# bababyVN/medical-image-segmentation-and-classification

Hardware: NVIDIA B200
Metric: AttU_Net 256x256 train images/sec (higher is better)
Workload: dtype bf16

## Files before the change

### include/b200seg.h

```cpp
#ifndef B200SEG_H_
#define B200SEG_H_

#include <stdint.h>

#ifdef __cplusplus
extern "C" {
#endif

#define B2_ABI_VERSION 1

enum {
  B2_OK = 0,
  B2_ERR_SHAPE = -1,
  B2_ERR_ALIGN = -2,
  B2_ERR_ARCH = -3,
  B2_ERR_CUDA = -4,
  B2_ERR_NCCL = -5,
  B2_ERR_WORKSPACE = -6
};

typedef void* b2_stream_t;

const char* b2_last_error(void);
int b2_abi_version(void);
int b2_arch_check(void);
int b2_num_sms(void);

int b2_set_deterministic(void* workspace, int64_t bytes);
int b2_get_deterministic(void);

int b2_reload_env(void);

typedef struct b2_conv_args {
  int32_t n, h, w;
  int32_t ksize;
  const void* x0;
  int32_t c0, ldx0;
  const void* x1;
  int32_t c1, ldx1;
  const void* wpk;
  int32_t ktot;
  int64_t w_tap_stride;
  int32_t cout;
  void* y;
  int32_t ldy;
  const float* bias;
  const void* addend;
  int32_t ldadd;
  double* stats;
  int32_t relu;
  int32_t stride;
  int32_t out_mul, out_off_h, out_off_w;
  int32_t in_mul, in_off_h, in_off_w;
  int32_t custom_pad, pad_h, pad_w;
  int32_t add_after_act;
  int32_t fold_mode;
} b2_conv_args;

int b2_conv_fprop(const b2_conv_args* a, b2_stream_t stream);
int b2_conv_dgrad(const b2_conv_args* a, b2_stream_t stream);

typedef struct b2_wgrad_args {
  int32_t n, h, w;
  int32_t ksize;
  const void* dy;
  int32_t cout, lddy;
  const void* x0;
  int32_t c0, ldx0;
  const void* x1;
  int32_t c1, ldx1;
  float* dw;
  int32_t accumulate;
  void* workspace;
  int64_t workspace_bytes;
  int32_t x_stride;
  int32_t dy_mul, dy_off_h, dy_off_w;
  int32_t custom_pad, pad_h, pad_w;
  int32_t fold;
} b2_wgrad_args;

int64_t b2_conv_wgrad_workspace(const b2_wgrad_args* a);
int b2_conv_wgrad(const b2_wgrad_args* a, b2_stream_t stream);
// ... 206 lines not shown
```

### medical-image-segmentation-and-classification_b200/b200seg/_lib.py

```python
from __future__ import annotations

import ctypes as C
import os
from pathlib import Path

_PKG_DIR = Path(__file__).resolve().parent
LIB_PATH = Path(os.environ.get("B200SEG_LIB", _PKG_DIR.parent / "lib" / "libb200seg.so"))

B2_OK = 0
ERR_NAMES = {-1: "B2_ERR_SHAPE", -2: "B2_ERR_ALIGN", -3: "B2_ERR_ARCH", -4: "B2_ERR_CUDA", -5: "B2_ERR_NCCL",
             -6: "B2_ERR_WORKSPACE"}

_vp, _i32, _i64, _f32 = C.c_void_p, C.c_int32, C.c_int64, C.c_float


class ConvArgs(C.Structure):
    _fields_ = [("n", _i32), ("h", _i32), ("w", _i32), ("ksize", _i32),
                ("x0", _vp), ("c0", _i32), ("ldx0", _i32),
                ("x1", _vp), ("c1", _i32), ("ldx1", _i32),
                ("wpk", _vp), ("ktot", _i32), ("w_tap_stride", _i64),
                ("cout", _i32), ("y", _vp), ("ldy", _i32),
                ("bias", _vp), ("addend", _vp), ("ldadd", _i32),
                ("stats", _vp), ("relu", _i32),
                ("stride", _i32), ("out_mul", _i32), ("out_off_h", _i32), ("out_off_w", _i32),
                ("in_mul", _i32), ("in_off_h", _i32), ("in_off_w", _i32),
                ("custom_pad", _i32), ("pad_h", _i32), ("pad_w", _i32), ("add_after_act", _i32),
                ("fold_mode", _i32)]


class WgradArgs(C.Structure):
    _fields_ = [("n", _i32), ("h", _i32), ("w", _i32), ("ksize", _i32),
                ("dy", _vp), ("cout", _i32), ("lddy", _i32),
                ("x0", _vp), ("c0", _i32), ("ldx0", _i32),
                ("x1", _vp), ("c1", _i32), ("ldx1", _i32),
                ("dw", _vp), ("accumulate", _i32),
                ("workspace", _vp), ("workspace_bytes", _i64), ("x_stride", _i32),
                ("dy_mul", _i32), ("dy_off_h", _i32), ("dy_off_w", _i32),
                ("custom_pad", _i32), ("pad_h", _i32), ("pad_w", _i32), ("fold", _i32)]


class BnRunRef(C.Structure):
    _fields_ = [("stats", _vp), ("running_mean", _vp), ("running_var", _vp), ("num_batches_tracked", _vp),
                ("count", _i64), ("c", _i32), ("momentum", C.c_float)]


class F32ConvArgs(C.Structure):
    _fields_ = [("x0", _vp), ("x1", _vp), ("c0", _i32), ("c1", _i32), ("ldx0", _i32), ("ldx1", _i32),
                ("n", _i32), ("hi", _i32), ("wi", _i32), ("ho", _i32), ("wo", _i32),
                ("ksize", _i32), ("stride", _i32), ("pad_h", _i32), ("pad_w", _i32),
                ("w", _vp), ("bias", _vp), ("addend", _vp),
                ("ldadd", _i32), ("add_after_act", _i32), ("relu", _i32), ("cout", _i32),
                ("y", _vp), ("ldy", _i32), ("out_mul", _i32), ("out_off_h", _i32), ("out_off_w", _i32)]


class GateArgs(C.Structure):
    _fields_ = [("n", _i32), ("h", _i32), ("w", _i32), ("c", _i32), ("fint", _i32),
                ("g", _vp), ("ldg", _i32), ("x", _vp), ("ldx", _i32),
                ("wpk", _vp), ("bias", _vp), ("wpsi", _vp), ("bpsi", _vp), ("scale1", _vp), ("shift1", _vp),
                ("out", _vp), ("ldo", _i32)]


class GateCoef(C.Structure):
    _fields_ = [(k, _vp) for k in (
        "scale_g", "shift_g", "mean_g", "invstd_g", "gamma_g",
        "scale_x", "shift_x", "mean_x", "invstd_x", "gamma_x",
        "gamma1", "mean1", "invstd1", "wpsi")]


SIGNATURES = {
    "b2_last_error": (C.c_char_p, []),
    "b2_abi_version": (C.c_int, []),
    "b2_arch_check": (C.c_int, []),
    "b2_num_sms": (C.c_int, []),
    "b2_set_deterministic": (C.c_int, [_vp, _i64]),
    "b2_get_deterministic": (C.c_int, []),
    "b2_reload_env": (C.c_int, []),
    "b2_conv_fprop": (C.c_int, [C.POINTER(ConvArgs), _vp]),
    "b2_conv_dgrad": (C.c_int, [C.POINTER(ConvArgs), _vp]),
    "b2_conv_wgrad_workspace": (_i64, [C.POINTER(WgradArgs)]),
    "b2_conv_wgrad": (C.c_int, [C.POINTER(WgradArgs), _vp]),
    "b2_pack_weights": (C.c_int, [_vp, _i32, _i32, _i32, _i64, _i64, _i64, _i64, _vp, _vp, _vp]),
    "b2_pack_weights_folded": (C.c_int, [_vp, _i32, _i32, _i32, _i64, _i64, _i64, _i64, _vp, _vp, _vp, _i32, _vp, _vp,
                                         _vp]),
    "b2_pack_weights_upfold": (C.c_int, [_vp, _i32, _i32, _i64, _i64, _i64, _i64, _vp, _vp, _vp]),
    "b2_fold_upconv_wgrad": (C.c_int, [_vp, _i32, _i32, _vp, _vp]),
    "b2_conv_smallc_fprop": (C.c_int, [_vp, _i32, _i32, _i32, _i32, _vp, _vp, _i32, _vp, _i32, _i32, _vp]),
    "b2_conv_smallc_wgrad": (C.c_int, [_vp, _i32, _vp, _i32, _i32, _i32, _i32, _i32, _vp, _vp]),
    "b2_head_fwd": (C.c_int, [_vp, _i32, _i64, _i32, _i32, _vp, _vp, _i32, _vp, _vp]),
    "b2_head_bwd": (C.c_int, [_vp, _vp, _i32, _i64, _i32, _i32, _vp, _i32, _vp, _i32, _vp, _vp, _vp]),
    "b2_channel_stats": (C.c_int, [_vp, _i32, _i64, _i32, _vp, _vp]),
    "b2_bn_finalize": (C.c_int, [_vp, _i32, _i64, _vp, _vp, _f32, _f32, _vp, _vp, _vp, _vp, _vp, _vp, _vp, _vp]),
    "b2_bn_update_running_multi": (C.c_int, [_vp, _i32, _i32, _vp]),
    "b2_bn_eval_coeffs": (C.c_int, [_vp, _vp, _vp, _vp, _f32, _i32, _vp, _vp, _vp, _vp, _vp]),
    "b2_bn_apply": (C.c_int, [_vp, _i32, _i64, _i32, _vp, _vp, _i32, _vp, _i32, _vp, _i32, _vp, _i32, _vp]),
    "b2_bn_bwd_reduce": (C.c_int, [_vp, _i32, _vp, _i32, _i64, _i32, _vp, _vp, _vp, _vp, _i32, _vp, _vp]),
    "b2_bn_bwd_apply": (C.c_int, [_vp, _i32, _vp, _i32, _i64, _i32, _vp, _vp, _vp, _vp, _vp, _i32, _i32, _vp,
                                  _vp, _i32, _vp, _vp, _vp, _vp]),
    "b2_channel_sum": (C.c_int, [_vp, _i32, _i64, _i32, _vp, _vp]),
    "b2_maxpool2x2_fwd": (C.c_int, [_vp, _i32, _i32, _i32, _i32, _i32, _vp, _i32, _vp]),
    "b2_maxpool2x2_bwd": (C.c_int, [_vp, _i32, _vp, _i32, _i32, _i32, _i32, _i32, _vp, _i32, _vp]),
    "b2_maxpool2x2_bwd_add": (C.c_int, [_vp, _i32, _vp, _i32, _i32, _i32, _i32, _i32, _vp, _i32, _vp, _i32, _vp]),
    "b2_upsample2x_fwd": (C.c_int, [_vp, _i32, _i32, _i32, _i32, _i32, _vp, _i32, _vp]),
    "b2_upsample2x_bwd": (C.c_int, [_vp, _i32, _i32, _i32, _i32, _i32, _vp, _i32, _vp]),
    "b2_add": (C.c_int, [_vp, _i32, _vp, _i32, _i64, _i32, _vp, _i32, _vp]),
    "b2_nchw_f32_to_nhwc_bf16": (C.c_int, [_vp, _i32, _i32, _i32, _i32, _vp, _i32, _vp]),
    "b2_stem_im2col3x3": (C.c_int, [_vp, _i32, _i32, _i32, _i32, _vp, _vp]),
    "b2_layout_nchw_to_nhwc": (C.c_int, [_vp, _i32, _i32, _i32, _i32, _vp, _i32, _vp]),
    "b2_layout_nhwc_to_nchw": (C.c_int, [_vp, _i32, _i32, _i32, _i32, _i32, _vp, _vp]),
    "b2_stem7x7_fprop": (C.c_int, [_vp, _i32, _i32, _i32, _vp, _i32, _vp, _i32, _vp]),
    "b2_maxpool3x3s2_fwd": (C.c_int, [_vp, _i32, _i32, _i32, _i32, _i32, _vp, _i32, _vp]),
    "b2_gate_psi_fwd": (C.c_int, [_vp, _vp, _i32, _i64, _i32, _vp, _vp, _vp, _vp, _vp, _vp, _vp, _vp, _vp]),
    "b2_gate_apply_fwd": (C.c_int, [_vp, _i32, _vp, _i64, _i32, _vp, _vp, _vp, _vp, _i32, _vp]),
    "b2_gate_apply_bwd": (C.c_int, [_vp, _i32, _vp, _i32, _vp, _vp, _i64, _i32, _vp, _vp, _vp, _i32, _vp, _vp,
                                    _vp]),
    "b2_gate_psi_bwd_reduce": (C.c_int, [_vp, _vp, _vp, _vp, _i32, _i64, _i32, C.POINTER(GateCoef), _vp, _i32,
                                         _vp, _vp, _vp, _vp]),
    "b2_gate_psi_bwd_apply": (C.c_int, [_vp, _vp, _vp, _vp, _i32, _i64, _i32, C.POINTER(GateCoef), _vp, _i32,
                                        _vp, _vp, _vp, _vp, _vp, _vp, _vp]),
    "b2_grad_sqnorm_multi": (C.c_int, [_vp, _vp, _vp, _i32, _i32, _vp, _vp, _vp]),
    "b2_adamw_multi": (C.c_int, [_vp, _vp, _vp, _i32, _i32, _vp, _f32, _vp, _f32, _f32, _f32, _f32, _vp, _vp, _vp]),
    "b2_pack_weights_multi": (C.c_int, [_vp, _i32, _i32, _vp]),
    "b2_seg_augment": (C.c_int, [_vp, _vp, _i32, _i32, _i32, _i32, _vp, C.POINTER(_f32), C.POINTER(_f32), _i32, _vp, _vp,
                                 _vp]),
    "b2_gate_fused": (C.c_int, [C.POINTER(GateArgs), _vp]),
    "b2_stem_im2col": (C.c_int, [_vp, _i32, _i32, _i32, _i32, _i32, _i32, _i32, _i32, _vp, _vp]),
    "b2_maxpool3x3s2_bwd": (C.c_int, [_vp, _i32, _vp, _i32, _i32, _i32, _i32, _i32, _vp, _i32, _vp]),
    "b2_zero_insert2x": (C.c_int, [_vp, _i32, _i32, _i32, _i32, _i32, _vp, _i32, _vp]),
# ... 66 lines not shown
```

### medical-image-segmentation-and-classification_b200/csrc/common.cuh

```cuda
#pragma once
#include <cuda.h>
#include <cuda_runtime.h>
#include <cuda_bf16.h>
#include <stdint.h>
#include <stdio.h>
#include <string.h>

#include "../../include/b200seg.h"

namespace b2 {

void set_error(const char* fmt, ...);
int  cuda_fail(cudaError_t e, const char* what);

#define B2_CHECK_CUDA(expr)                                            \
  do {                                                                 \
    cudaError_t _e = (expr);                                           \
    if (_e != cudaSuccess) return ::b2::cuda_fail(_e, #expr);          \
  } while (0)

#define B2_REQUIRE(cond, code, ...)                                    \
  do {                                                                 \
    if (!(cond)) { ::b2::set_error(__VA_ARGS__); return (code); }      \
  } while (0)
// ... 4 lines not shown

int env_switch(const char* name, int dflt);

__device__ __forceinline__ void pdl_wait() { asm volatile("griddepcontrol.wait;" ::: "memory"); }
__device__ __forceinline__ void pdl_trigger() { asm volatile("griddepcontrol.launch_dependents;" ::: "memory"); }
__device__ __forceinline__ void pdl_enter() {
  pdl_wait();
  pdl_trigger();
}

inline bool pdl_allowed(long long work_bytes) {
  const int mode = env_switch("B200SEG_PDL", 2);
  if (mode == 0) return false;
  if (mode == 1) return true;
  return work_bytes <= (long long)env_switch("B200SEG_PDL_MB", 16) * (1ll << 20);
}

template <typename... KArgs, typename... Args>
inline cudaError_t launch_chain(void (*kernel)(KArgs...), dim3 grid, dim3 block, size_t smem, cudaStream_t stream,
                                int cluster, long long work_bytes, Args&&... args) {
  cudaLaunchConfig_t cfg = {};
  cfg.gridDim = grid;
  cfg.blockDim = block;
  cfg.dynamicSmemBytes = smem;
  cfg.stream = stream;
  cudaLaunchAttribute at[2];
  unsigned n = 0;
  if (cluster > 1) {
    at[n].id = cudaLaunchAttributeClusterDimension;
    at[n].val.clusterDim.x = (unsigned)cluster;
    at[n].val.clusterDim.y = 1;
    at[n].val.clusterDim.z = 1;
    ++n;
  }
  if (pdl_allowed(work_bytes)) {
    at[n].id = cudaLaunchAttributeProgrammaticStreamSerialization;
    at[n].val.programmaticStreamSerializationAllowed = 1;
    ++n;
  }
  cfg.attrs = at;
  cfg.numAttrs = n;
  return cudaLaunchKernelEx(&cfg, kernel, static_cast<KArgs>(args)...);
}

int encode_tmap_bf16(CUtensorMap* out, const void* base, int rank, const uint64_t* dims,
                     const uint64_t* strides_bytes, const uint32_t* box, CUtensorMapSwizzle swz,
                     const uint32_t* elem_strides = nullptr);

struct DetBuf {
  double* partial;
  int n;
};
int det_begin(DetBuf* out, long long rows, int n, cudaStream_t stream, long long keep = 0);
int det_finish(const double* partial, long long rows, int row_stride, int count, double* dst, cudaStream_t stream);
int det_finish(const double* partial, long long rows, int row_stride, int count, float* dst, cudaStream_t stream);
bool det_enabled();

#ifdef __CUDACC__
template <typename T>
__device__ __forceinline__ void red_out(T* dst, const DetBuf& d, int idx, T v) {
  if (d.partial != nullptr) d.partial[(size_t)blockIdx.x * d.n + idx] = (double)v;
  else atomicAdd(dst + idx, v);
}
__device__ __forceinline__ uint32_t smem_u32(const void* p) {
  return (uint32_t)__cvta_generic_to_shared(p);
}

__device__ __forceinline__ void mbar_init(uint64_t* bar, uint32_t count) {
  asm volatile("mbarrier.init.shared::cta.b64 [%0], %1;" ::"r"(smem_u32(bar)), "r"(count) : "memory");
}
__device__ __forceinline__ void fence_barrier_init() {
  asm volatile("fence.mbarrier_init.release.cluster;" ::: "memory");
}
__device__ __forceinline__ void fence_proxy_async() {
  asm volatile("fence.proxy.async.shared::cta;" ::: "memory");
}
__device__ __forceinline__ void mbar_arrive_expect_tx(uint64_t* bar, uint32_t bytes) {
  asm volatile("mbarrier.arrive.expect_tx.shared::cta.b64 _, [%0], %1;" ::"r"(smem_u32(bar)), "r"(bytes)
               : "memory");
}
__device__ __forceinline__ void mbar_arrive(uint64_t* bar) {
  asm volatile("mbarrier.arrive.shared::cta.b64 _, [%0];" ::"r"(smem_u32(bar)) : "memory");
}
__device__ __forceinline__ bool mbar_try_wait(uint64_t* bar, uint32_t parity) {
  uint32_t ok;
  asm volatile(
      "{\n\t.reg .pred p;\n\t"
      "mbarrier.try_wait.parity.shared::cta.b64 p, [%1], %2;\n\t"
      "selp.u32 %0, 1, 0, p;\n\t}"
      : "=r"(ok)
      : "r"(smem_u32(bar)), "r"(parity)
      : "memory");
  return ok != 0;
}
__device__ __forceinline__ void mbar_wait(uint64_t* bar, uint32_t parity) {
  uint32_t spins = 0;
  while (!mbar_try_wait(bar, parity)) {
    if (++spins > (1u << 26)) { __trap(); }
  }
}

__device__ __forceinline__ void tma_load_2d(void* smem, const CUtensorMap* tm, uint64_t* bar, int c0, int c1) {
  asm volatile(
      "cp.async.bulk.tensor.2d.shared::cluster.global.mbarrier::complete_tx::bytes [%0], [%1, {%3, %4}], [%2];"
      ::"r"(smem_u32(smem)), "l"(reinterpret_cast<uint64_t>(tm)), "r"(smem_u32(bar)), "r"(c0), "r"(c1)
      : "memory");
// ... 227 lines not shown
```

### medical-image-segmentation-and-classification_b200/csrc/conv_igemm.cu

```cuda
#include <stdlib.h>
#include <mutex>

#include "common.cuh"
#include "igemm_util.cuh"

namespace b2 {

static constexpr int kMaxEpiGroups = 2;
static constexpr int kThreads = 64 + 128 * kMaxEpiGroups;
static constexpr int kMaxStages = 12;

struct IgemmParams {
  int H, W, N;
  int Wb, Hb, Nb;
  int tw, th;
  int taps;
  int cb0, cb1;
  int block_n, stages, num_k_iters;
  int cout, n_tiles, m_tiles, m_stride;
  int halo, base_off_mode;
  int dm;
  int rp;
  int stride, ksize, pad_h, pad_w;
  long long y_sn, y_sh, y_sw;
// ... 290 lines not shown
#pragma unroll
                  for (int k = 0; k < kKBlock / 16; ++k)
                    umma_bf16(d_tmem, desc_hi | (uint64_t)(a_lo + 2 * k), desc_hi | (uint64_t)(b_lo + 2 * k), idesc,
                              (it | s | k) != 0 ? 1u : 0u);
                }
                a_lo += 8;
                b_lo += b_tap_step;
              }
            }
          } else {
          const uint32_t d_tmem = tmem_base + (uint32_t)((ti & 1) * p.block_n);
          for (int s = 0; s < ((p.debug_skip & 2) ? 0 : sub); ++s) {
            const uint32_t a_s = a_addr + s * 128;
            const uint32_t b_s = b_addr + s * p.block_n * 128;
            const uint32_t bo = p.base_off_mode ? ((a_s >> 7) & 7u) : 0u;
#pragma unroll
            for (int k = 0; k < kKBlock / 16; ++k) {
              const uint64_t da = umma_desc_sw128_bo(a_s + k * 32, 16, 1024, bo);
              const uint64_t db = umma_desc_sw128(b_s + k * 32, 16, 1024);
              umma_bf16(d_tmem, da, db, idesc, (it | s | k) != 0 ? 1u : 0u);
            }
          }
          }
          if constexpr (kPair) {
            umma_commit_pair(&empty_bar[stage], 3);
          } else {
            if (C == 1) umma_commit(&empty_bar[stage]);
            else umma_commit_mc(&empty_bar[stage], cmask);
          }
        }
        __syncwarp();
        if (++stage == p.stages) {
          stage = 0;
          phase ^= 1;
        }
      }
      if (elect_one()) {
        for (int q = 0; q < a_slots; ++q) {
          uint64_t* fb = &tmem_full_bar[(uint32_t)(a_slots * ti + q) & (uint32_t)(nbuf - 1)];
          if constexpr (kPair) umma_commit_pair(fb, 3);
          else umma_commit(fb);
        }
      }
      __syncwarp();
    }
  } else if (warp >= 2 && ((warp - 2) >> 2) < p.epi_groups) {
    const int g = (warp - 2) >> 2;
    const int G = p.epi_groups;
    const int et = (threadIdx.x - 64) & 127;
    uint8_t* ctile = ctile0 + g * ctile_bytes;
    float* s_bias = s_bias0 + g * 256;
    float* s_psi = s_psi0 + g * 256;
    const int bar_id = 1 + g;
    const int quad = warp & 3;
    const int row = quad * 32 + lane;
    const int wl = row % p.Wb;
    const int hl = (row / p.Wb) % p.Hb;
    const int nl = row / (p.Wb * p.Hb);
    const bool relu = p.relu != 0;
    const int nchunks = p.block_n >> 3;
    const int schunk = lane % nchunks;
    const int sgrp = et / nchunks;
    double acc[16];
#pragma unroll
    for (int i = 0; i < 16; ++i) acc[i] = 0.0;
    const int fold_tiles = 32 / nchunks;
    float fs[8], fq[8];
#pragma unroll
    for (int j = 0; j < 8; ++j) fs[j] = fq[j] = 0.f;
    int fpending = 0;
    auto fold_stats = [&]() {
#pragma unroll
      for (int j = 0; j < 8; ++j) {
        acc[j] += (double)fs[j];
        acc[8 + j] += (double)fq[j];
        fs[j] = fq[j] = 0.f;
      }
      fpending = 0;
    };

    auto flush_stats = [&](int n_tile_) {
      fold_stats();
      for (int off = nchunks; off < 32; off <<= 1) {
#pragma unroll
        for (int i = 0; i < 16; ++i) acc[i] += __shfl_xor_sync(0xffffffffu, acc[i], off);
      }
      if (p.tma_store && et == 0) tma_store_wait_read();
      asm volatile("bar.sync %0, 128;" ::"r"(bar_id) : "memory");
      double* red = reinterpret_cast<double*>(ctile);
      if (lane < nchunks) {
        double* r0 = red + ((warp - 2) & 3) * 2 * p.block_n + schunk * 8;
#pragma unroll
        for (int j = 0; j < 8; ++j) {
          r0[j] = acc[j];
          r0[p.block_n + j] = acc[8 + j];
        }
      }
      asm volatile("bar.sync %0, 128;" ::"r"(bar_id) : "memory");
      for (int i = et; i < 2 * p.block_n; i += 128) {
        const int which = i / p.block_n, c = i % p.block_n;
        double v = 0.0;
#pragma unroll
        for (int w = 0; w < 4; ++w) v += red[(w * 2 + which) * p.block_n + c];
        const int sidx = which * p.cout + n_tile_ * p.block_n + (p.rp ? (c & 63) : c);
        if (p.stats_partial != nullptr)
          p.stats_partial[(size_t)(blockIdx.x * p.epi_groups + g) * (2 * p.cout) + sidx] += v;
// ... 740 lines not shown
```

### medical-image-segmentation-and-classification_b200/csrc/conv_small.cu

```cuda
#include "common.cuh"

namespace b2 {

template <int KS>
__global__ void __launch_bounds__(128) smallc_fprop_kernel(const uint2* __restrict__ x4, int n, int h, int w,
                                                           const float* __restrict__ wk,
                                                           const float* __restrict__ bias, int cout,
                                                           __nv_bfloat16* __restrict__ y, int ldy, int relu) {
  constexpr int TAPS = KS * KS;
  extern __shared__ float sm[];
  float* sw = sm;
  float* sb = sm + cout * TAPS * 4;
  for (int i = threadIdx.x; i < cout * TAPS * 4; i += blockDim.x) sw[i] = bf16_round(wk[i]);
  for (int i = threadIdx.x; i < cout; i += blockDim.x) sb[i] = bias ? bias[i] : 0.f;
  __syncthreads();
  const long long total = (long long)n * h * w;
  for (long long p = (long long)blockIdx.x * blockDim.x + threadIdx.x; p < total;
       p += (long long)gridDim.x * blockDim.x) {
    const int xx = (int)(p % w);
    const int yy = (int)((p / w) % h);
    float in[TAPS][4];
#pragma unroll
    for (int t = 0; t < TAPS; ++t) {
      const int dy = (KS == 3) ? t / 3 - 1 : 0, dx = (KS == 3) ? t % 3 - 1 : 0;
// ... 287 lines not shown
    smallc_wgrad_kernel<3><<<(unsigned)grid, 256, 0, (cudaStream_t)stream>>>((const __nv_bfloat16*)dy, lddy,
                                                                             (const uint2*)x4, n, h, w, dw, det);
  else
    smallc_wgrad_kernel<1><<<(unsigned)grid, 256, 0, (cudaStream_t)stream>>>((const __nv_bfloat16*)dy, lddy,
                                                                             (const uint2*)x4, n, h, w, dw, det);
  B2_LAUNCH_CHECK();
  if (det.partial) return det_finish(det.partial, grid, det.n, ncol, dw, (cudaStream_t)stream);
  return B2_OK;
}

extern "C" int b2_head_fwd(const void* x, int32_t ldx, int64_t npix, int32_t hw, int32_t cin, const float* w,
                           const float* bias, int32_t cout, float* y, b2_stream_t stream) {
  B2_REQUIRE(cin % 8 == 0 && cin <= 256, B2_ERR_SHAPE, "head cin=%d must be a multiple of 8, <= 256", cin);
  B2_REQUIRE(cout >= 1 && cout <= 8, B2_ERR_SHAPE, "head cout=%d must be in 1..8", cout);
  B2_REQUIRE(npix > 0 && npix < (1ll << 31) && hw > 0, B2_ERR_SHAPE, "head: pixel count out of range");
  B2_REQUIRE(ldx % 8 == 0 && (reinterpret_cast<uintptr_t>(x) & 15) == 0, B2_ERR_ALIGN, "x misaligned");
  const int L = pow2ceil(cin / 8);
  const int gpb = 256 / L;
  long long grid = (npix + gpb - 1) / gpb;
  const long long cap = (long long)num_sms() * 8;
  if (grid > cap) grid = cap;
#define B2_HEAD_FWD(CO) head_fwd_kernel<CO><<<(unsigned)grid, 256, 0, (cudaStream_t)stream>>>( \
      (const __nv_bfloat16*)x, ldx, npix, hw, cin, w, bias, cout, L, y)
  if (cout == 1) B2_HEAD_FWD(1); else if (cout == 2) B2_HEAD_FWD(2); else if (cout <= 4) B2_HEAD_FWD(4); else B2_HEAD_FWD(8);
#undef B2_HEAD_FWD
  B2_LAUNCH_CHECK();
  return B2_OK;
}

extern "C" int b2_head_bwd(const float* dy, const void* x, int32_t ldx, int64_t npix, int32_t hw, int32_t cin,
                           const float* w, int32_t cout, void* dx, int32_t lddx, float* dw, float* db,
                           b2_stream_t stream) {
  B2_REQUIRE(cin % 8 == 0 && cin <= 256, B2_ERR_SHAPE, "head cin=%d must be a multiple of 8, <= 256", cin);
  B2_REQUIRE(cout >= 1 && cout <= 8, B2_ERR_SHAPE, "head cout=%d must be in 1..8", cout);
  B2_REQUIRE(npix > 0 && npix < (1ll << 31) && hw > 0, B2_ERR_SHAPE, "head: pixel count out of range");
  B2_REQUIRE(ldx % 8 == 0 && (reinterpret_cast<uintptr_t>(x) & 15) == 0, B2_ERR_ALIGN, "x misaligned");
  B2_REQUIRE(dx == nullptr || (lddx % 8 == 0 && (reinterpret_cast<uintptr_t>(dx) & 15) == 0), B2_ERR_ALIGN,
             "dx misaligned");
  const int L = pow2ceil(cin / 8);
  const int gpb = 256 / L;
  long long grid = (npix + gpb - 1) / gpb;
  const long long cap = (long long)num_sms() * 6;
  if (grid > cap) grid = cap;
  const size_t smem = (size_t)(cout * cin + cout) * sizeof(float);
  DetBuf det;
  int rc = det_begin(&det, grid, cout * cin + cout, (cudaStream_t)stream);
  if (rc) return rc;
#define B2_HEAD_BWD(CO) head_bwd_kernel<CO><<<(unsigned)grid, 256, smem, (cudaStream_t)stream>>>( \
      dy, (const __nv_bfloat16*)x, ldx, npix, hw, cin, w, cout, L, (__nv_bfloat16*)dx, lddx, dw, db, det)
  if (cout == 1) B2_HEAD_BWD(1); else if (cout == 2) B2_HEAD_BWD(2); else if (cout <= 4) B2_HEAD_BWD(4); else B2_HEAD_BWD(8);
#undef B2_HEAD_BWD
  B2_LAUNCH_CHECK();
  if (det.partial) {
    rc = det_finish(det.partial, grid, det.n, cout * cin, dw, (cudaStream_t)stream);
    if (rc) return rc;
    return det_finish(det.partial + cout * cin, grid, det.n, cout, db, (cudaStream_t)stream);
  }
  return B2_OK;
}
```

### medical-image-segmentation-and-classification_b200/csrc/gate.cu

```cuda
#include <stdlib.h>

#include "common.cuh"

namespace b2 {

__device__ __forceinline__ void g_unpack8(const uint4& u, float* f) {
  f[0] = bf16lo(u.x); f[1] = bf16hi(u.x); f[2] = bf16lo(u.y); f[3] = bf16hi(u.y);
  f[4] = bf16lo(u.z); f[5] = bf16hi(u.z); f[6] = bf16lo(u.w); f[7] = bf16hi(u.w);
}
__device__ __forceinline__ uint4 g_pack8(const float* f) {
  return make_uint4(pack_bf16x2(f[0], f[1]), pack_bf16x2(f[2], f[3]), pack_bf16x2(f[4], f[5]),
                    pack_bf16x2(f[6], f[7]));
}
__device__ __forceinline__ void g_load8(const float* p, bool has, float* f) {
#pragma unroll
  for (int j = 0; j < 8; ++j) f[j] = has ? __ldg(p + j) : 0.f;
}
__device__ __forceinline__ float sigmoidf_(float x) { return 1.f / (1.f + expf(-x)); }

__device__ __forceinline__ void block_sum2_out(float a, float b, double* dst, const DetBuf& det) {
  __shared__ float sh[2][8];
  a = warp_sum(a);
  b = warp_sum(b);
  const int warp = threadIdx.x >> 5, lane = threadIdx.x & 31;
// ... 501 lines not shown
  B2_CHECK_CUDA(launch_chain(gate_apply_bwd_kernel, dim3(grid), dim3(256), (size_t)(0), (cudaStream_t)stream, 1,
      (long long)npix * c * 2, (const __nv_bfloat16*)dout, lddout, (const __nv_bfloat16*)x, ldx,
      (const __nv_bfloat16*)psi, (const __nv_bfloat16*)q, npix, c / 8, L, mean1, invstd1, (__nv_bfloat16*)dx, lddx,
      dsig, sums1, det));
  B2_LAUNCH_CHECK();
  if (det.partial) return det_finish(det.partial, grid, det.n, 2, sums1, (cudaStream_t)stream);
  return B2_OK;
}

static GateBwdCoef make_coef(const b2_gate_coef* k) {
  GateBwdCoef c;
  c.scale_g = k->scale_g; c.shift_g = k->shift_g; c.mean_g = k->mean_g; c.invstd_g = k->invstd_g;
  c.gamma_g = k->gamma_g;
  c.scale_x = k->scale_x; c.shift_x = k->shift_x; c.mean_x = k->mean_x; c.invstd_x = k->invstd_x;
  c.gamma_x = k->gamma_x;
  c.gamma1 = k->gamma1; c.mean1 = k->mean1; c.invstd1 = k->invstd1;
  c.wpsi = k->wpsi;
  return c;
}

extern "C" int b2_gate_psi_bwd_reduce(const float* dsig, const void* q, const void* g1p, const void* x1p,
                                      int32_t ld, int64_t npix, int32_t fint, const b2_gate_coef* coef,
                                      const double* sums1, int32_t training, double* sums, float* dwpsi,
                                      float* dbpsi, b2_stream_t stream) {
  B2_REQUIRE(fint % 8 == 0 && fint <= 256, B2_ERR_SHAPE, "F_int=%d must be a multiple of 8, <= 256", fint);
  B2_REQUIRE(g_al(g1p, ld) && g_al(x1p, ld), B2_ERR_ALIGN, "gate operands misaligned");
  const bool light = gate_light(fint);
  const int slice = (light && fint > 64 && env_switch("B200SEG_GATE_SLICE", 1) != 0) ? 64 : 0;
  const int slices = slice ? (fint + slice - 1) / slice : 1;
  const size_t smem = (size_t)(4 * (slice ? slice : fint) + 1) * sizeof(float);
  const int L = g_pow2ceil((slice ? slice : fint) / (light ? 4 : 8));
  int grid = g_grid(npix, 256 / L, light ? 8 : 4);
  grid = (grid + slices - 1) / slices;
  DetBuf det;
  int rc = det_begin(&det, grid, 5 * fint + 1, (cudaStream_t)stream);
  if (rc) return rc;
  if (light && env_switch("B200SEG_GATE_U", fint <= 128 ? 4 : 2) == 4) {
    B2_CHECK_CUDA(launch_chain(gate_psi_bwd_reduce_kernel<4, 4, 2>, dim3(grid, slices), dim3(256), (size_t)(smem),
        (cudaStream_t)stream, 1, (long long)npix * fint * 2, dsig, (const __nv_bfloat16*)q, (const __nv_bfloat16*)g1p,
        (const __nv_bfloat16*)x1p, ld, npix, fint, L, make_coef(coef), sums1, training, sums, dwpsi, dbpsi, slice,
        det));
  } else if (light) {
    B2_CHECK_CUDA(launch_chain(gate_psi_bwd_reduce_kernel<4, 2, 3>, dim3(grid, slices), dim3(256), (size_t)(smem),
        (cudaStream_t)stream, 1, (long long)npix * fint * 2, dsig, (const __nv_bfloat16*)q, (const __nv_bfloat16*)g1p,
        (const __nv_bfloat16*)x1p, ld, npix, fint, L, make_coef(coef), sums1, training, sums, dwpsi, dbpsi, slice,
        det));
  } else {
    B2_CHECK_CUDA(launch_chain(gate_psi_bwd_reduce_kernel<8, 2, 2>, dim3(grid), dim3(256), (size_t)(smem),
        (cudaStream_t)stream, 1, (long long)npix * fint * 2, dsig, (const __nv_bfloat16*)q, (const __nv_bfloat16*)g1p,
        (const __nv_bfloat16*)x1p, ld, npix, fint, L, make_coef(coef), sums1, training, sums, dwpsi, dbpsi, 0, det));
  }
  B2_LAUNCH_CHECK();
  if (det.partial) {
    rc = det_finish(det.partial, grid, det.n, 4 * fint, sums, (cudaStream_t)stream);
    if (rc) return rc;
    rc = det_finish(det.partial + 4 * fint, grid, det.n, fint, dwpsi, (cudaStream_t)stream);
    if (rc) return rc;
    return det_finish(det.partial + 5 * fint, grid, det.n, 1, dbpsi, (cudaStream_t)stream);
  }
  return B2_OK;
}

extern "C" int b2_gate_psi_bwd_apply(const float* dsig, const void* q, const void* g1p, const void* x1p,
                                     int32_t ld, int64_t npix, int32_t fint, const b2_gate_coef* coef,
                                     const double* sums1, int32_t training, const double* sums, void* dg1p,
                                     void* dx1p, float* dgamma_beta, float* dbn1, float* dbias,
                                     b2_stream_t stream) {
  B2_REQUIRE(fint % 8 == 0 && fint <= 256, B2_ERR_SHAPE, "F_int=%d must be a multiple of 8, <= 256", fint);
  B2_REQUIRE(g_al(g1p, ld) && g_al(x1p, ld) && g_al(dg1p, ld) && g_al(dx1p, ld), B2_ERR_ALIGN,
             "gate operands misaligned");
  const bool light = gate_light(fint);
  int tpp = fint / (light ? 4 : 8), slices = 1;
  if (light && fint > 64 && env_switch("B200SEG_GATE_SLICE", 1) != 0) {
    tpp = 16;
    slices = (fint + 63) / 64;
  }
  const int rows = 256 / tpp;
  int grid = g_grid(npix, rows, 8);
  grid = (grid + slices - 1) / slices;
  DetBuf det;
  det.partial = nullptr;
  det.n = 2 * fint;
  if (dbias != nullptr) {
    int rc = det_begin(&det, grid, 2 * fint, (cudaStream_t)stream);
    if (rc) return rc;
  }
  if (light && env_switch("B200SEG_GATE_U", fint <= 128 ? 4 : 2) == 4) {
    B2_CHECK_CUDA(launch_chain(gate_psi_bwd_apply_kernel<4, 4, 2>, dim3(grid, slices), dim3(256), (size_t)(0),
        (cudaStream_t)stream, 1, (long long)npix * fint * 2, dsig, (const __nv_bfloat16*)q, (const __nv_bfloat16*)g1p,
        (const __nv_bfloat16*)x1p, ld, npix, fint, tpp, rows, make_coef(coef), sums1, training, sums,
        (__nv_bfloat16*)dg1p, (__nv_bfloat16*)dx1p, dgamma_beta, dbn1, dbias, det));
  } else if (light) {
    B2_CHECK_CUDA(launch_chain(gate_psi_bwd_apply_kernel<4, 2, 3>, dim3(grid, slices), dim3(256), (size_t)(0),
        (cudaStream_t)stream, 1, (long long)npix * fint * 2, dsig, (const __nv_bfloat16*)q, (const __nv_bfloat16*)g1p,
        (const __nv_bfloat16*)x1p, ld, npix, fint, tpp, rows, make_coef(coef), sums1, training, sums,
        (__nv_bfloat16*)dg1p, (__nv_bfloat16*)dx1p, dgamma_beta, dbn1, dbias, det));
  } else {
    B2_CHECK_CUDA(launch_chain(gate_psi_bwd_apply_kernel<8, 2, 2>, dim3(grid), dim3(256), (size_t)(0),
        (cudaStream_t)stream, 1, (long long)npix * fint * 2, dsig, (const __nv_bfloat16*)q, (const __nv_bfloat16*)g1p,
        (const __nv_bfloat16*)x1p, ld, npix, fint, tpp, rows, make_coef(coef), sums1, training, sums,
        (__nv_bfloat16*)dg1p, (__nv_bfloat16*)dx1p, dgamma_beta, dbn1, dbias, det));
  }
  B2_LAUNCH_CHECK();
  if (det.partial) return det_finish(det.partial, grid, det.n, 2 * fint, dbias, (cudaStream_t)stream);
  return B2_OK;
}
```

### medical-image-segmentation-and-classification_b200/csrc/host_util.cu

```cuda
#include <stdarg.h>
#include <stdlib.h>
#include <map>
#include <mutex>
#include <string>

#include "common.cuh"

namespace b2 {

static thread_local char g_err[512] = "";

void set_error(const char* fmt, ...) {
  va_list ap;
  va_start(ap, fmt);
  vsnprintf(g_err, sizeof(g_err), fmt, ap);
  va_end(ap);
}

int cuda_fail(cudaError_t e, const char* what) {
  set_error("CUDA error %d (%s) at %s", (int)e, cudaGetErrorString(e), what);
  return B2_ERR_CUDA;
}

int num_sms() {
  static int cached[64] = {0};
  int dev = 0;
  if (cudaGetDevice(&dev) != cudaSuccess || dev < 0 || dev >= 64) return 148;
  if (cached[dev] == 0) {
    int n = 0;
    if (cudaDeviceGetAttribute(&n, cudaDevAttrMultiProcessorCount, dev) != cudaSuccess || n <= 0) n = 148;
    cached[dev] = n;
  }
  return cached[dev];
}

static std::mutex g_env_mu;
static std::map<std::string, int> g_env_cache;

int env_switch(const char* name, int dflt) {
  std::lock_guard<std::mutex> lk(g_env_mu);
  auto it = g_env_cache.find(name);
  if (it != g_env_cache.end()) return it->second == INT32_MIN ? dflt : it->second;
  const char* v = getenv(name);
  const int val = v ? atoi(v) : INT32_MIN;
  g_env_cache.emplace(name, val);
  return v ? val : dflt;
}

static std::mutex g_det_mu;
static double* g_det_ws[64] = {nullptr};
static long long g_det_doubles[64] = {0};

static bool det_lookup(double** ws, long long* n) {
  int dev = 0;
  if (cudaGetDevice(&dev) != cudaSuccess || dev < 0 || dev >= 64) return false;
  std::lock_guard<std::mutex> lk(g_det_mu);
  *ws = g_det_ws[dev];
  *n = g_det_doubles[dev];
  return *ws != nullptr;
}

bool det_enabled() {
  double* ws;
  long long n;
  return det_lookup(&ws, &n);
}

int det_begin(DetBuf* out, long long rows, int n, cudaStream_t stream, long long keep) {
  out->partial = nullptr;
  out->n = n;
  double* ws;
  long long cap;
  if (!det_lookup(&ws, &cap)) return B2_OK;
  const long long need = rows * (long long)n;
  B2_REQUIRE(keep + need <= cap, B2_ERR_WORKSPACE,
             "deterministic workspace too small: need %lld B, have %lld B (b2_set_deterministic)",
             (keep + need) * 8, cap * 8);
  out->partial = ws + keep;
  B2_CHECK_CUDA(cudaMemsetAsync(out->partial, 0, (size_t)need * sizeof(double), stream));
  return B2_OK;
}

template <typename T>
__global__ void det_finish_kernel(const double* __restrict__ partial, long long rows, int row_stride, int count,
                                  T* __restrict__ dst) {
  const int i = blockIdx.x * blockDim.x + threadIdx.x;
  if (i >= count) return;
  double s = 0.0;
  for (long long r = 0; r < rows; ++r) s += partial[r * row_stride + i];
  dst[i] = (T)((double)dst[i] + s);
}

int det_finish(const double* partial, long long rows, int row_stride, int count, double* dst, cudaStream_t stream) {
  if (count <= 0) return B2_OK;
  det_finish_kernel<double><<<(count + 127) / 128, 128, 0, stream>>>(partial, rows, row_stride, count, dst);
  B2_LAUNCH_CHECK();
  return B2_OK;
}
int det_finish(const double* partial, long long rows, int row_stride, int count, float* dst, cudaStream_t stream) {
  if (count <= 0) return B2_OK;
  det_finish_kernel<float><<<(count + 127) / 128, 128, 0, stream>>>(partial, rows, row_stride, count, dst);
  B2_LAUNCH_CHECK();
  return B2_OK;
}

typedef CUresult (*EncodeTiledFn)(CUtensorMap*, CUtensorMapDataType, cuuint32_t, void*, const cuuint64_t*,
                                  const cuuint64_t*, const cuuint32_t*, const cuuint32_t*, CUtensorMapInterleave,
                                  CUtensorMapSwizzle, CUtensorMapL2promotion, CUtensorMapFloatOOBfill);

static EncodeTiledFn get_encode_fn() {
  static EncodeTiledFn fn = nullptr;
  static std::once_flag once;
  std::call_once(once, [] {
    void* p = nullptr;
    cudaDriverEntryPointQueryResult q;
    if (cudaGetDriverEntryPoint("cuTensorMapEncodeTiled", &p, cudaEnableDefault, &q) == cudaSuccess &&
        q == cudaDriverEntryPointSuccess) {
      fn = reinterpret_cast<EncodeTiledFn>(p);
    }
  });
  return fn;
}

int encode_tmap_bf16(CUtensorMap* out, const void* base, int rank, const uint64_t* dims,
                     const uint64_t* strides_bytes, const uint32_t* box, CUtensorMapSwizzle swz,
                     const uint32_t* elem_strides) {
  EncodeTiledFn fn = get_encode_fn();
  B2_REQUIRE(fn != nullptr, B2_ERR_CUDA, "cuTensorMapEncodeTiled entry point unavailable (no driver?)");
  B2_REQUIRE((reinterpret_cast<uintptr_t>(base) & 15) == 0, B2_ERR_ALIGN, "TMA base pointer not 16B aligned");
  cuuint64_t gdim[5];
  cuuint64_t gstr[5];
  cuuint32_t bdim[5];
  cuuint32_t estr[5];
  for (int i = 0; i < rank; ++i) {
    gdim[i] = dims[i];
    bdim[i] = box[i];
    estr[i] = elem_strides ? elem_strides[i] : 1;
    if (i > 0) {
      gstr[i - 1] = strides_bytes[i];
      B2_REQUIRE((strides_bytes[i] & 15) == 0, B2_ERR_ALIGN, "TMA stride %d = %llu B not a multiple of 16", i,
                 (unsigned long long)strides_bytes[i]);
    }
  }
  CUresult r = fn(out, CU_TENSOR_MAP_DATA_TYPE_BFLOAT16, (cuuint32_t)rank, const_cast<void*>(base), gdim, gstr,
                  bdim, estr, CU_TENSOR_MAP_INTERLEAVE_NONE, swz, CU_TENSOR_MAP_L2_PROMOTION_L2_256B,
                  CU_TENSOR_MAP_FLOAT_OOB_FILL_NONE);
  if (r != CUDA_SUCCESS) {
    set_error("cuTensorMapEncodeTiled failed (%d): rank %d dims [%llu,%llu,%llu,%llu] box [%u,%u,%u,%u]", (int)r,
              rank, (unsigned long long)dims[0], (unsigned long long)(rank > 1 ? dims[1] : 0),
              (unsigned long long)(rank > 2 ? dims[2] : 0), (unsigned long long)(rank > 3 ? dims[3] : 0), box[0],
              rank > 1 ? box[1] : 0, rank > 2 ? box[2] : 0, rank > 3 ? box[3] : 0);
    return B2_ERR_CUDA;
  }
  return B2_OK;
}

}

extern "C" {

const char* b2_last_error(void) { return b2::g_err; }
int b2_abi_version(void) { return B2_ABI_VERSION; }
int b2_num_sms(void) { return b2::num_sms(); }

int b2_set_deterministic(void* workspace, int64_t bytes) {
  int dev = 0;
  cudaError_t e = cudaGetDevice(&dev);
  if (e != cudaSuccess) return b2::cuda_fail(e, "cudaGetDevice");
  B2_REQUIRE(dev >= 0 && dev < 64, B2_ERR_SHAPE, "device index %d out of range", dev);
  B2_REQUIRE(workspace == nullptr || (bytes >= (1 << 20) && (reinterpret_cast<uintptr_t>(workspace) & 15) == 0),
             B2_ERR_WORKSPACE, "deterministic workspace must be 16 B aligned and >= 1 MiB");
  std::lock_guard<std::mutex> lk(b2::g_det_mu);
  b2::g_det_ws[dev] = static_cast<double*>(workspace);
  b2::g_det_doubles[dev] = workspace ? bytes / 8 : 0;
  return B2_OK;
}

int b2_get_deterministic(void) { return b2::det_enabled() ? 1 : 0; }

int b2_reload_env(void) {
  std::lock_guard<std::mutex> lk(b2::g_env_mu);
  b2::g_env_cache.clear();
  return B2_OK;
}

int b2_arch_check(void) {
  int dev = 0;
  cudaError_t e = cudaGetDevice(&dev);
  if (e != cudaSuccess) return b2::cuda_fail(e, "cudaGetDevice");
  int major = 0, minor = 0;
  e = cudaDeviceGetAttribute(&major, cudaDevAttrComputeCapabilityMajor, dev);
  if (e != cudaSuccess) return b2::cuda_fail(e, "cudaDeviceGetAttribute");
  cudaDeviceGetAttribute(&minor, cudaDevAttrComputeCapabilityMinor, dev);
  if (major != 10 || minor != 0) {
    b2::set_error("libb200seg is built for sm_100a only; device %d is sm_%d%d", dev, major, minor);
    return B2_ERR_ARCH;
  }
  return B2_OK;
}

}
```

Baseline: 1986.

## Batch deterministic reduction finishes into one segmented kernel and drop workspace memset

Replaces the per-output det_finish launches with a single segmented kernel. It covers up to four destinations, stages row chunks through double-buffered shared memory and is launched with programmatic dependent launch. It also removes the cudaMemsetAsync of the partial workspace, and the igemm epilogue now zeroes its own stats rows. The aim is to cut launch count and memset traffic, but this only affects deterministic mode. Any kernel that does not fully write its partial rows could now read stale data.

```diff
diff --git a/include/b200seg.h b/include/b200seg.h
--- a/include/b200seg.h
+++ b/include/b200seg.h
@@ -28,6 +28,8 @@
 
 int b2_set_deterministic(void* workspace, int64_t bytes);
 int b2_get_deterministic(void);
+int b2_det_finish(const double* partial, int64_t rows, int32_t row_stride, int32_t nseg, const int32_t* offsets,
+                  const int32_t* counts, void* const* dsts, const int32_t* dst_f64, b2_stream_t stream);
 
 int b2_reload_env(void);
 
diff --git a/medical-image-segmentation-and-classification_b200/b200seg/_lib.py b/medical-image-segmentation-and-classification_b200/b200seg/_lib.py
--- a/medical-image-segmentation-and-classification_b200/b200seg/_lib.py
+++ b/medical-image-segmentation-and-classification_b200/b200seg/_lib.py
@@ -73,6 +73,7 @@
     "b2_arch_check": (C.c_int, []),
     "b2_num_sms": (C.c_int, []),
     "b2_set_deterministic": (C.c_int, [_vp, _i64]),
+    "b2_det_finish": (C.c_int, [_vp, _i64, _i32, _i32, _vp, _vp, _vp, _vp, _vp]),
     "b2_get_deterministic": (C.c_int, []),
     "b2_reload_env": (C.c_int, []),
     "b2_conv_fprop": (C.c_int, [C.POINTER(ConvArgs), _vp]),
diff --git a/medical-image-segmentation-and-classification_b200/csrc/common.cuh b/medical-image-segmentation-and-classification_b200/csrc/common.cuh
--- a/medical-image-segmentation-and-classification_b200/csrc/common.cuh
+++ b/medical-image-segmentation-and-classification_b200/csrc/common.cuh
@@ -80,6 +80,16 @@
   int n;
 };
 int det_begin(DetBuf* out, long long rows, int n, cudaStream_t stream, long long keep = 0);
+static constexpr int kDetMaxSeg = 4;
+struct DetSeg {
+  int offset;
+  int count;
+  void* dst;
+  int f64;
+};
+inline DetSeg det_seg(int offset, int count, double* dst) { return DetSeg{offset, count, dst, 1}; }
+inline DetSeg det_seg(int offset, int count, float* dst) { return DetSeg{offset, count, dst, 0}; }
+int det_finish(const double* partial, long long rows, int row_stride, const DetSeg* seg, int nseg, cudaStream_t stream);
 int det_finish(const double* partial, long long rows, int row_stride, int count, double* dst, cudaStream_t stream);
 int det_finish(const double* partial, long long rows, int row_stride, int count, float* dst, cudaStream_t stream);
 bool det_enabled();
diff --git a/medical-image-segmentation-and-classification_b200/csrc/conv_igemm.cu b/medical-image-segmentation-and-classification_b200/csrc/conv_igemm.cu
--- a/medical-image-segmentation-and-classification_b200/csrc/conv_igemm.cu
+++ b/medical-image-segmentation-and-classification_b200/csrc/conv_igemm.cu
@@ -366,6 +366,11 @@
     float* s_bias = s_bias0 + g * 256;
     float* s_psi = s_psi0 + g * 256;
     const int bar_id = 1 + g;
+    if (p.stats_partial != nullptr) {
+      double* srow = p.stats_partial + (size_t)(blockIdx.x * G + g) * (2 * p.cout);
+      for (int i = et; i < 2 * p.cout; i += 128) srow[i] = 0.0;
+      asm volatile("bar.sync %0, 128;" ::"r"(bar_id) : "memory");
+    }
     const int quad = warp & 3;
     const int row = quad * 32 + lane;
     const int wl = row % p.Wb;
diff --git a/medical-image-segmentation-and-classification_b200/csrc/conv_small.cu b/medical-image-segmentation-and-classification_b200/csrc/conv_small.cu
--- a/medical-image-segmentation-and-classification_b200/csrc/conv_small.cu
+++ b/medical-image-segmentation-and-classification_b200/csrc/conv_small.cu
@@ -363,9 +363,8 @@
 #undef B2_HEAD_BWD
   B2_LAUNCH_CHECK();
   if (det.partial) {
-    rc = det_finish(det.partial, grid, det.n, cout * cin, dw, (cudaStream_t)stream);
-    if (rc) return rc;
-    return det_finish(det.partial + cout * cin, grid, det.n, cout, db, (cudaStream_t)stream);
+    const DetSeg seg[2] = {det_seg(0, cout * cin, dw), det_seg(cout * cin, cout, db)};
+    return det_finish(det.partial, grid, det.n, seg, 2, (cudaStream_t)stream);
   }
   return B2_OK;
 }
diff --git a/medical-image-segmentation-and-classification_b200/csrc/gate.cu b/medical-image-segmentation-and-classification_b200/csrc/gate.cu
--- a/medical-image-segmentation-and-classification_b200/csrc/gate.cu
+++ b/medical-image-segmentation-and-classification_b200/csrc/gate.cu
@@ -577,11 +577,8 @@
   }
   B2_LAUNCH_CHECK();
   if (det.partial) {
-    rc = det_finish(det.partial, grid, det.n, 4 * fint, sums, (cudaStream_t)stream);
-    if (rc) return rc;
-    rc = det_finish(det.partial + 4 * fint, grid, det.n, fint, dwpsi, (cudaStream_t)stream);
-    if (rc) return rc;
-    return det_finish(det.partial + 5 * fint, grid, det.n, 1, dbpsi, (cudaStream_t)stream);
+    const DetSeg seg[3] = {det_seg(0, 4 * fint, sums), det_seg(4 * fint, fint, dwpsi), det_seg(5 * fint, 1, dbpsi)};
+    return det_finish(det.partial, grid, det.n, seg, 3, (cudaStream_t)stream);
   }
   return B2_OK;
 }
diff --git a/medical-image-segmentation-and-classification_b200/csrc/host_util.cu b/medical-image-segmentation-and-classification_b200/csrc/host_util.cu
--- a/medical-image-segmentation-and-classification_b200/csrc/host_util.cu
+++ b/medical-image-segmentation-and-classification_b200/csrc/host_util.cu
@@ -67,6 +67,7 @@
 }
 
 int det_begin(DetBuf* out, long long rows, int n, cudaStream_t stream, long long keep) {
+  (void)stream;
   out->partial = nullptr;
   out->n = n;
   double* ws;
@@ -77,31 +78,111 @@
              "deterministic workspace too small: need %lld B, have %lld B (b2_set_deterministic)",
              (keep + need) * 8, cap * 8);
   out->partial = ws + keep;
-  B2_CHECK_CUDA(cudaMemsetAsync(out->partial, 0, (size_t)need * sizeof(double), stream));
-  return B2_OK;
-}
-
-template <typename T>
-__global__ void det_finish_kernel(const double* __restrict__ partial, long long rows, int row_stride, int count,
-                                  T* __restrict__ dst) {
-  const int i = blockIdx.x * blockDim.x + threadIdx.x;
-  if (i >= count) return;
-  double s = 0.0;
-  for (long long r = 0; r < rows; ++r) s += partial[r * row_stride + i];
-  dst[i] = (T)((double)dst[i] + s);
-}
-
+  return B2_OK;
+}
+
+static constexpr int kFinThreads = 256;
+static constexpr int kFinChunk = 3072;
+static constexpr int kFinLoads = kFinChunk / kFinThreads;
+
+struct DetFinishJob {
+  const double* partial;
+  long long rows;
+  int row_stride;
+  int nseg;
+  DetSeg seg[kDetMaxSeg];
+  int first_block[kDetMaxSeg + 1];
+};
+
+__global__ void __launch_bounds__(kFinThreads) det_finish_kernel(DetFinishJob j) {
+  __shared__ double buf[2][kFinChunk];
+  pdl_enter();
+  int s = 0;
+  while (s + 1 < j.nseg && (int)blockIdx.x >= j.first_block[s + 1]) ++s;
+  const DetSeg sg = j.seg[s];
+  const int c0 = ((int)blockIdx.x - j.first_block[s]) * 32;
+  const int w = sg.count - c0 < 32 ? sg.count - c0 : 32;
+  const int ch = kFinChunk / w;
+  const int per = ch * w;
+  const long long rows = j.rows;
+  const double* src = j.partial + sg.offset + c0;
+  int er[kFinLoads], eo[kFinLoads];
+#pragma unroll
+  for (int k = 0; k < kFinLoads; ++k) {
+    const int e = k * kFinThreads + (int)threadIdx.x;
+    er[k] = e < per ? e / w : INT32_MAX;
+    eo[k] = e < per ? er[k] * j.row_stride + (e - er[k] * w) : 0;
+  }
+  double v[kFinLoads];
+  auto load = [&](long long r0) {
+    const double* base = src + r0 * j.row_stride;
+#pragma unroll
+    for (int k = 0; k < kFinLoads; ++k) v[k] = r0 + er[k] < rows ? __ldg(base + eo[k]) : 0.0;
+  };
+  auto stash = [&](double* b) {
+#pragma unroll
+    for (int k = 0; k < kFinLoads; ++k)
+      if (k * kFinThreads + (int)threadIdx.x < per) b[k * kFinThreads + threadIdx.x] = v[k];
+  };
+  const long long nchunks = (rows + ch - 1) / ch;
+  load(0);
+  stash(buf[0]);
+  __syncthreads();
+  double acc = 0.0;
+  for (long long q = 0; q < nchunks; ++q) {
+    if (q + 1 < nchunks) load((q + 1) * ch);
+    if ((int)threadIdx.x < w) {
+      const double* b = buf[q & 1] + threadIdx.x;
+      const int n = rows - q * ch < ch ? (int)(rows - q * ch) : ch;
+#pragma unroll 8
+      for (int r = 0; r < n; ++r) acc += b[r * w];
+    }
+    if (q + 1 < nchunks) stash(buf[(q + 1) & 1]);
+    __syncthreads();
+  }
+  if ((int)threadIdx.x < w) {
+    const int i = c0 + (int)threadIdx.x;
+    if (sg.f64) {
+      double* d = static_cast<double*>(sg.dst);
+      d[i] = d[i] + acc;
+    } else {
+      float* d = static_cast<float*>(sg.dst);
+      d[i] = (float)((double)d[i] + acc);
+    }
+  }
+}
+
+int det_finish(const double* partial, long long rows, int row_stride, const DetSeg* seg, int nseg,
+               cudaStream_t stream) {
+  B2_REQUIRE(nseg >= 1 && nseg <= kDetMaxSeg && rows >= 1, B2_ERR_SHAPE, "det_finish: %d segments, %lld rows",
+             nseg, rows);
+  DetFinishJob j;
+  j.partial = partial;
+  j.rows = rows;
+  j.row_stride = row_stride;
+  j.nseg = nseg;
+  int blocks = 0;
+  for (int s = 0; s < nseg; ++s) {
+    B2_REQUIRE(seg[s].count >= 0 && seg[s].offset >= 0 && seg[s].offset + seg[s].count <= row_stride, B2_ERR_SHAPE,
+               "det_finish: segment %d (offset %d, count %d) outside a row of %d", s, seg[s].offset, seg[s].count,
+               row_stride);
+    j.seg[s] = seg[s];
+    j.first_block[s] = blocks;
+    blocks += (seg[s].count + 31) / 32;
+  }
+  j.first_block[nseg] = blocks;
+  if (blocks == 0) return B2_OK;
+  B2_CHECK_CUDA(launch_chain(det_finish_kernel, dim3(blocks), dim3(kFinThreads), (size_t)0, stream, 1,
+                             rows * row_stride * (long long)sizeof(double), j));
+  return B2_OK;
+}
 int det_finish(const double* partial, long long rows, int row_stride, int count, double* dst, cudaStream_t stream) {
-  if (count <= 0) return B2_OK;
-  det_finish_kernel<double><<<(count + 127) / 128, 128, 0, stream>>>(partial, rows, row_stride, count, dst);
-  B2_LAUNCH_CHECK();
-  return B2_OK;
+  const DetSeg s = det_seg(0, count, dst);
+  return det_finish(partial, rows, row_stride, &s, 1, stream);
 }
 int det_finish(const double* partial, long long rows, int row_stride, int count, float* dst, cudaStream_t stream) {
-  if (count <= 0) return B2_OK;
-  det_finish_kernel<float><<<(count + 127) / 128, 128, 0, stream>>>(partial, rows, row_stride, count, dst);
-  B2_LAUNCH_CHECK();
-  return B2_OK;
+  const DetSeg s = det_seg(0, count, dst);
+  return det_finish(partial, rows, row_stride, &s, 1, stream);
 }
 
 typedef CUresult (*EncodeTiledFn)(CUtensorMap*, CUtensorMapDataType, cuuint32_t, void*, const cuuint64_t*,
@@ -178,6 +259,15 @@
 
 int b2_get_deterministic(void) { return b2::det_enabled() ? 1 : 0; }
 
+int b2_det_finish(const double* partial, int64_t rows, int32_t row_stride, int32_t nseg, const int32_t* offsets,
+                  const int32_t* counts, void* const* dsts, const int32_t* dst_f64, b2_stream_t stream) {
+  B2_REQUIRE(nseg >= 1 && nseg <= b2::kDetMaxSeg, B2_ERR_SHAPE, "b2_det_finish: %d segments (1..%d)", nseg,
+             b2::kDetMaxSeg);
+  b2::DetSeg seg[b2::kDetMaxSeg];
+  for (int s = 0; s < nseg; ++s) seg[s] = {offsets[s], counts[s], dsts[s], dst_f64[s] != 0 ? 1 : 0};
+  return b2::det_finish(partial, rows, row_stride, seg, nseg, (cudaStream_t)stream);
+}
+
 int b2_reload_env(void) {
   std::lock_guard<std::mutex> lk(b2::g_env_mu);
   b2::g_env_cache.clear();
```

Measured after the change: 2118 (median of 6 runs). 1.07x the previous value.
